# torchmd/torchmd-net

Measured on AMD Instinct MI355X. Metric: molecules/sec (64-atom molecules) TensorNet E+F, higher is better.
Workload: dtype f32; 1 GPU; BASELINE configs[1]: TensorNet F=128 L=2 K=32 rc=5.0, S-mol64 256 molecules x 64 atoms per GPU, energies + forces, random-init weights (seed 0); atoms_per_gpu=16384, pairs_per_gpu=193709, directed_edges_per_gpu=403802, parallelism=molecule-sharded x1, RCCL all-reduce of energies, rank_step=eager: tmdnet_build_graph (pair-count read-back) + tmdnet_energy_forces

## Files before the change

__graft_entry__.py:

```python
import os
import subprocess
import sys

ROOT = os.path.dirname(os.path.abspath(__file__))
PKG_DIR = os.path.join(ROOT, "torchmd-net_amd")
CSRC = os.path.join(PKG_DIR, "csrc")
LIB_DIR = os.path.join(PKG_DIR, "lib")
LIB = os.path.join(LIB_DIR, "libtmdnet_amd.so")
HIP_SOURCES = ["tn_api.hip", "tn_gemm.hip", "tn_gemm_skinny.hip", "tn_gemm_dual.hip", "tn_gemm_sb.hip", "tn_gemm_sb1.hip", "tn_tlin9.hip", "tn_small.hip", "tn_mid.hip", "tn_pairgrad.hip", "tn_kernels.hip", "tn_message_pair.hip", "tn_edge_table.hip", "tn_embed_rb.hip", "tn_train.hip", "tn_hvp.hip", "tn_et_hvp.hip", "tn_tn2_hvp.hip", "tn_hvp_api.hip", "tn_tn2.hip", "tn_tn2_api.hip", "tn_graph_wave.hip", "tn_neighbors_f64.hip", "tn_cell.hip", "tn_et.hip", "tn_et_g16.hip", "tn_et_api.hip", "tn_heads.hip", "tn_virial.hip"]

if PKG_DIR not in sys.path:
    sys.path.insert(0, PKG_DIR)
if ROOT not in sys.path:
    sys.path.insert(0, ROOT)


def _newer(target, sources):
    if not os.path.exists(target):
        return True
    t = os.path.getmtime(target)
    return any(os.path.getmtime(s) > t for s in sources)


def build_hip(force=False, verbose=True):
    from concurrent.futures import ThreadPoolExecutor

    os.makedirs(LIB_DIR, exist_ok=True)
    obj_dir = os.path.join(PKG_DIR, "build")
    os.makedirs(obj_dir, exist_ok=True)
    srcs = [os.path.join(CSRC, s) for s in HIP_SOURCES]
    headers = [os.path.join(CSRC, h) for h in os.listdir(CSRC) if h.endswith(".h")]
    headers.append(os.path.join(ROOT, "include", "tmdnet_amd.h"))
    hipcc = os.environ.get("HIPCC", "/opt/rocm/bin/hipcc")
    flags = ["--offload-arch=gfx950", "-O3", "-std=c++17", "-fPIC", "-Wno-unused-value", "-I" + os.path.join(ROOT, "include")]
    objs, todo = [], []
    for src in srcs:
        obj = os.path.join(obj_dir, os.path.basename(src)[:-4] + ".o")
        objs.append(obj)
        if force or _newer(obj, [src] + headers):
            todo.append((src, obj))

    def compile_one(job):
        src, obj = job
        cmd = [hipcc] + flags + ["-c", src, "-o", obj]
        if verbose:
            print("[build]", " ".join(cmd), flush=True)
        subprocess.check_call(cmd)

    if todo:
# ... 54 lines not shown
```

torchmd-net_amd/csrc/tn_api.hip:

```cpp
#include <hip/hip_runtime.h>

#include <algorithm>
#include <cmath>
#include <cstdio>
#include <cstdlib>
#include <cstring>
#include <map>
#include <unordered_map>
#include <string>
#include <vector>

#include "tn_heads.h"
#include "tn_model.h"
#include "tn_tlin9.h"
#include "tn_small.h"
#include "tn_interp.h"
#include "tn_virial.h"

using namespace tn;

static const char* kCatNames[CAT_COUNT] = {"graph", "gemm_edge", "gemm_node", "message", "pair_bwd", "embed_scatter", "elementwise", "edge_table"};

int fail(tmdnet_model* m, int code, const std::string& msg) {
  if (m) m->err = msg;
  return code;
}
// ... 872 lines not shown
      for (int l = 0; l <= L; ++l) {
        const std::string t = "cp" + std::to_string(l) + ".";
        add_sb(t + "W1", F, 3 * F);
        add_sb(t + "W1T", 3 * F, F);
        add_sb(t + "W2", F, F);
        add_sb(t + "W2T", F, F);
        add_sb(t + "W3", 2 * qd, F);
        add_sb(t + "W3T", F, 2 * qd);
      }
    }
    add_sb("Lin", F, 3 * F);
    add_sb("LinT", 3 * F, F);
    add_sb("O1", H, F);
    add_sb("O1T", F, H);
    std::vector<Img> fms;
    auto add_fm = [&](const std::string& key) {
      if (F % 32) return;
      fms.push_back({key, F, F, sb_elems});
      sb_elems += split_weight_fm_elems(F, F);
    };
    for (int k = 0; k < 3; ++k) {
      add_fm("Ue" + std::to_string(k));
      add_fm("UeT" + std::to_string(k));
    }
    for (int l = 0; l < L; ++l)
      for (int k = 0; k < 6; ++k) {
        add_fm("l" + std::to_string(l) + ".V" + std::to_string(k));
        add_fm("l" + std::to_string(l) + ".VT" + std::to_string(k));
      }
    if (m->dev_sb && m->dev_sb_cap < sb_elems) {
      HIP_TRY(m, hipFree(m->dev_sb));
      m->dev_sb = nullptr;
    }
    if (!m->dev_sb) {
      HIP_TRY(m, hipMalloc(reinterpret_cast<void**>(&m->dev_sb), sb_elems * sizeof(uint16_t)));
      m->dev_sb_cap = sb_elems;
    }
    for (const auto& im : imgs) launch_split_weight_tiles(m->dev + off.at(im.key), im.n, im.k, m->dev_sb + im.o, nullptr);
    for (const auto& im : fms) launch_split_weight_fm(m->dev + off.at(im.key), im.n, im.k, m->dev_sb + im.o, nullptr);
    m->image_jobs.clear();
    for (const auto& im : imgs) m->image_jobs.push_back({off.at(im.key), im.n, im.k, im.o, 0});
    for (const auto& im : fms) m->image_jobs.push_back({off.at(im.key), im.n, im.k, im.o, 1});
    m->packed_elems = pk.buf.size();
    m->sb_of.clear();
// ... 131 lines not shown
  HIP_TRY(m, hipGetLastError());
  return TMDNET_OK;
}

int tmdnet_set_option(tmdnet_model* m, const char* name, double value) {
  if (!m || !name) return TMDNET_ERR_INVALID;
  const std::string n(name);
  if (n == "edge_table_min_pairs") {
    m->tab_min_pairs = value < 0 ? 0 : (int64_t)value;
    return TMDNET_OK;
  }
  if (n == "embed_rb_min_atoms") {
    m->rb_min_atoms = value < 0 ? 0 : (int64_t)value;
    return TMDNET_OK;
  }
  if (n == "pair_rows_bf16") {
    if (!m->et) return fail(m, TMDNET_ERR_INVALID, "pair_rows_bf16 applies to the Equivariant Transformer handle only");
    m->pair_bf16 = value != 0.0 ? 1 : 0;
    return TMDNET_OK;
  }
  if (n == "recompute_pair_rows") {
    if (m->et || m->tn2) return fail(m, TMDNET_ERR_INVALID, "recompute_pair_rows applies to the TensorNet handle only");
    m->recompute_rows = value != 0.0;
    return TMDNET_OK;
  }
  return fail(m, TMDNET_ERR_INVALID, "unknown option: " + n);
}

int tmdnet_get_info(const tmdnet_model* m, const char* name, double* value) {
  if (!m || !name || !value) return TMDNET_ERR_INVALID;
  const std::string n(name);
  if (m->tabs_pending && n.rfind("edge_table_", 0) == 0 && n != "edge_table_min_pairs")
    if (const int rc = ensure_radial_tables(const_cast<tmdnet_model*>(m), nullptr)) return rc;
  if (n == "edge_table_T") *value = m->tabs.ok ? m->tabs.T : 0;
  else if (n == "edge_table_err_value") *value = m->tabs.err_value;
  else if (n == "edge_table_err_slope") *value = m->tabs.err_slope;
  else if (n == "edge_table_min_pairs") *value = (double)m->tab_min_pairs;
  else if (n == "pair_rows_bf16") *value = (double)m->pair_bf16;
  else if (n == "embed_rb_min_atoms") *value = (double)m->rb_min_atoms;
  else if (n == "recompute_pair_rows") *value = m->recompute_rows ? 1.0 : 0.0;
  else if (n == "embed_rb") *value = m->rb_fwd ? 1.0 : 0.0;
  else if (n == "species_last_build") *value = (double)m->last_nt;
  else if (n == "halo_active_first") *value = (double)m->halo_active[0];
  else if (n == "halo_active_rows") *value = (double)m->halo_active[1];
  else return TMDNET_ERR_INVALID;
  return TMDNET_OK;
}

int tmdnet_set_cell_grid(tmdnet_model* m, int32_t ncx, int32_t ncy, int32_t ncz) {
  if (!m) return TMDNET_ERR_INVALID;
  if (ncx < 0 || ncy < 0 || ncz < 0) ncx = ncy = ncz = -1;
  m->cell_n[0] = ncx;
  m->cell_n[1] = ncy;
  m->cell_n[2] = ncz;
// ... 307 lines not shown
    if (h[2] > 0 && h[2] < N && h[1] - h[0] + 1 == h[2] && images && tlin9_ok(h[2], F, true)) {
      a0 = h[0];
      Na = h[2];
    }
  }
  const bool rng = Na != N;
  const bool t9 = !tc && tlin9_ok(Na, F, rng) && tlin9_images(W.Ue) && tlin9_images(W.UeT) && (L == 0 || tlin9_images(W.layer[0].V));
  const bool t9r = !tc && L > 0 && tlin9_ok(Na, F, rng) && tlin9_images(W.UeT) && tlin9_images(W.layer[0].VT);
  m->halo_active[0] = a0;
  m->halo_active[1] = Na;
  const int64_t o1_ = a0, oF = (int64_t)a0 * F, o2F = 2 * oF, o3F = 3 * oF, o9F = 9 * oF, oH = (int64_t)a0 * H;
  const float* const q_a = q ? q + o1_ : nullptr;
  const int64_t* const batch_a = batch_k ? batch_k + o1_ : nullptr;
  const bool fused_small = !tc && !ntp && !recompute && !m->halo_fn && !m->head_kind && (small_fused_ok(N, F, H, L) || mid_fused_ok(N, F, H, L)) &&
                           (!want_forces || (message_adjoint_gd_ok(N, F) && !getenv("TMDNET_SEPARATE_PAIR_GD")));
  if (run_fwd) {
    if (use_tab) {
      const float* tabs[8];
      float* outs[8];
      float* douts[8];
      int nt_ = 0;
      if (!ntp) {
        tabs[nt_] = m->tabs.tab[0];
        outs[nt_] = b.Q;
        douts[nt_++] = want_forces ? b.dQ : nullptr;
      }
      for (int l = 0; l < L && !recompute; ++l) {
        tabs[nt_] = m->tabs.tab[1 + l];
        outs[nt_] = b.w[l];
        douts[nt_++] = want_forces ? b.dw[l] : nullptr;
// ... 66 lines not shown
        la.bO2 = W.bO2; la.atomref = W.atomref; la.Lin = W.Lin; la.O1 = W.O1; la.std_ = W.std;
        la.xhr = b.xhr; la.rstdr = b.rstdr; la.al = b.al; la.x = b.x; la.ea = b.ea;
        if (want_forces) { la.G = b.G; la.gMi = b.gMi; la.gPn = b.gPn; }
        KR(CAT_MESSAGE, wB + idxB + 6 * nodeB, (use_mid ? launch_mid_layer(la, last, s) : launch_small_layer(la, last, s)));
      }
      if (!want_forces) KR(CAT_ELEMENTWISE, Nd * 4, launch_mol_sum(g, b.ea, batch, N, B, W.mean, energy, s));
    } else {
    if (ntp) {
      KR(CAT_SCATTER, E_ * 12 + Pd * 48 + momB,
         (launch_pair_scalars(g, P, hp.cutoff_lower, hp.cutoff_upper, b.ps, s), launch_embed_moments(g, N, rbp, ntp, b.ps, b.mom, s)));
      KR(CAT_SCATTER, momB + Nd * 10 * Fd * 4, launch_embed_combine(g, N, F, K, ntp, z, W.Utab, W.Vtab, m->rb_fwd, b.mom, b.u0, b.s0n, s));
    } else {
      KR(CAT_SCATTER, Pd * 12 * Fd + E_ * 12 + Nd * 10 * Fd * 4,
         launch_embed_scatter(g, N, F, z, W.Utab, W.Vtab, b.Q, b.C, b.u0, b.s0n, s));
    }
    KR(CAT_ELEMENTWISE, Nd * Fd * 12,
       launch_layernorm_fwd(b.s0n + oF, W.ln0_w, W.ln0_b, Na, F, b.ln0 + oF, b.xh0 + oF, b.rstd0 + o1_, s));
    NODE();
    gemm(s, b.ln0 + oF, F, W.L1, F, W.bL1, b.h1 + o2F, 2 * F, Na, 2 * F, F, GEMM_ACT_SILU, b.a1 + o2F, 2 * F);
    gemm(s, b.h1 + o2F, 2 * F, W.L2, 2 * F, W.bL2, b.gates + o3F, 3 * F, Na, 3 * F, 2 * F, GEMM_ACT_SILU, b.a2 + o3F, 3 * F);
    if (t9) {
      Tl9Args ta{};
      ta.A = b.u0 + o9F; ta.C = b.X[0] + o9F; ta.o1 = b.UX + o9F; ta.e3 = b.gates + o3F; ta.N = Na; ta.F = F;
      tlin9(s, TL9_PRO_PLAIN, TL9_EPI_MULGATE, W.Ue, ta, 3.0 + 1.0 / 3.0, "gate");
    } else
      tensor_linear(s, b.u0, W.Ue, b.X[0], N, F, GEMM_MUL_AUX, b.UX, b.gates);
    for (int l = 0; l < L; ++l) {
      const LayerP& q_ = W.layer[l];
      if (es != s) HIP_TRY(m, hipStreamWaitEvent(s, m->ev_join[l], 0));
      float* const Xh_l = tc ? tc->Xh[l] : b.Xh;
      float* const Ch_l = tc ? tc->Ch[l] : b.Ch;
      float* const Xh_n = tc && l + 1 < L ? tc->Xh[l + 1] : b.Xh;
      if (t9) {
        Tl9Args ta{};
        ta.A = b.X[l] + o9F; ta.C = b.Pn[l] + o9F; ta.N = Na; ta.F = F;
// ... 5 lines not shown
        tb.A = Ch_l + o9F; tb.C = b.D[l] + o9F; tb.e0 = b.X[l] + o9F; tb.o1 = b.X[l + 1] + o9F; tb.o2 = b.feat + o3F;
        tb.want_feat = l + 1 == L; tb.kap = q_a;
        tb.N = Na; tb.F = F;
        tlin9(s, TL9_PRO_PLAIN, TL9_EPI_UPDATE, q_.V + 3, tb, 4.0 + (l + 1 == L ? 1.0 / 3.0 : 0.0), "update");
        continue;
      }
      if (l == 0) KR(CAT_ELEMENTWISE, 2 * nodeB, launch_norm_x(b.X[l], Xh_l, N, F, s));
      tensor_linear(s, Xh_l, q_.V, b.Pn[l], N, F);
      HALO_TRY(l, b.Pn[l], 9 * F);
      KR(CAT_MESSAGE, wB + idxB + 3 * nodeB, launch_message(g, N, F, b.w[l], b.Pn[l], q, batch_k, o3, b.Mi[l], Ch_l, s, recompute ? &rts[l] : nullptr));
      tensor_linear(s, Ch_l, q_.V + 3, b.D[l], N, F);
      KR(CAT_ELEMENTWISE, 4 * nodeB, launch_layer_update(Xh_l, b.D[l], q, batch_k, N, F, b.X[l + 1], l + 1 < L ? 1 : 2,
                                                         l + 1 < L ? Xh_n : b.feat, s));
    }
    if (L == 0) KR(CAT_ELEMENTWISE, nodeB + Nd * 3 * Fd * 4, launch_readout_feat(b.X[L] + o9F, Na, F, b.feat + o3F, s));
    KR(CAT_ELEMENTWISE, Nd * 3 * Fd * 12,
       launch_layernorm_fwd(b.feat + o3F, W.lnr_w, W.lnr_b, Na, 3 * F, b.lnr + o3F, b.xhr + o3F, b.rstdr + o1_, s));
    NODE();
    gemm(s, b.lnr + o3F, 3 * F, W.Lin, 3 * F, W.bLin, b.x + oF, F, Na, F, 3 * F, GEMM_ACT_SILU, b.al + oF, F);
    gemm(s, b.x + oF, F, W.O1, F, W.bO1, b.ao + oH, H, Na, H, F);
    if (m->head_kind) {
      KR(CAT_ELEMENTWISE, Nd * H * 4,
         launch_head_energy(b.ao, W.O2, W.bO2, N, H, W.std, nullptr, z, b.ea, s, want_forces ? b.g_ao : nullptr));
      heads.state = want_forces ? hbuf.state : nullptr;
      KR(CAT_ELEMENTWISE, Nd * 32, launch_heads_reduce(g, heads, hbuf, s));
    } else if ((int64_t)N <= 256 * (int64_t)B) {
      KR(CAT_ELEMENTWISE, Nd * H * 4, launch_head_mol_sum(g, b.ao, W.O2, W.bO2, N, B, H, W.std, W.atomref, z, batch, W.mean, energy, s,
                                                          want_forces ? b.g_ao : nullptr, m->atom_w, perm));
    } else {
      if (Na != N) launch_fill(b.ea, 0.f, N, s);
      KR(CAT_ELEMENTWISE, Nd * H * 4,
         launch_head_energy(b.ao + oH, W.O2, W.bO2, Na, H, W.std, W.atomref, z + o1_, b.ea + o1_, s, want_forces ? b.g_ao + oH : nullptr,
                            perm ? m->atom_w : (m->atom_w ? m->atom_w + o1_ : nullptr), perm ? perm + o1_ : nullptr));
      KR(CAT_ELEMENTWISE, Nd * 4, launch_mol_sum(g, b.ea, batch, N, B, W.mean, energy, s));
    }
    }
  }
  if (m->head_kind && want_forces && run_bwd)
    KR(CAT_ELEMENTWISE, Nd * (8 * H + 40), launch_heads_seed(heads, H, b.g_ao, hbuf.direct, s));

  if (want_forces && run_bwd && fused_small) {
    const int gd_nw = message_adjoint_gd_waves(g, N, F, recompute);
    const int64_t gd_stride = 2 * (int64_t)P1;
    for (int l = L - 1; l >= 0; --l) {
      const LayerP& q_ = W.layer[l];
      float* const gMi_in = ((L - 1 - l) & 1) ? b.gCh : b.gMi;
      float* const gMi_out = ((L - 1 - l) & 1) ? b.gMi : b.gCh;
      SmallRevArgs ra{};
      ra.g = g; ra.N = N; ra.F = F; ra.B = B; ra.o3 = o3; ra.first = l == 0; ra.kap = q;
// ... 22 lines not shown
    const RowMap rH = rows_plain(H), rF = rows_plain(F), r2F = rows_plain(2 * F), r3F = rows_plain(3 * F), rK = rows_plain(K);
    const RowMap rc_[3] = {rows_comp(F, 1), rows_comp(F, 3), rows_comp(F, 5)};
    const int c0_[3] = {0, 1, 4}, nc_[3] = {1, 3, 5};
    auto tensor_linear_grad = [&](const float* gOut, const float* In, const std::string& key) {
      for (int t = 0; t < 3; ++t)
        launch_tn_gemm(s, gOut + (int64_t)c0_[t] * F, rc_[t], In + (int64_t)c0_[t] * F, rc_[t], nullptr, nullptr, N * nc_[t], F, F,
                       tc->at(key + std::to_string(t)), false, tc->part);
    };
    if (tc) {
      launch_train_seed(b.ao, tc->gE, batch, N, H, W.std, b.g_ao, tc->head, s);
      launch_colsum(s, tc->head, rows_plain(H + 1), nullptr, rH, nullptr, nullptr, N, H, tc->at("O2"), false, tc->part);
      launch_colsum(s, tc->head + H, rows_plain(H + 1), nullptr, rH, nullptr, nullptr, N, 1, tc->at("bO2"), false, tc->part);
      launch_tn_gemm(s, b.g_ao, rH, b.x, rF, nullptr, nullptr, N, H, F, tc->at("O1"), false, tc->part);
      launch_colsum(s, b.g_ao, rH, nullptr, rH, nullptr, nullptr, N, H, tc->at("bO1"), false, tc->part);
    }
    gemm(s, b.g_ao + oH, H, W.O1T, H, nullptr, b.g_al + oF, F, Na, F, H, GEMM_MUL_DSILU_AUX, nullptr, 0, b.al + oF, F);
    gemm(s, b.g_al + oF, F, W.LinT, F, nullptr, b.g_ln + o3F, 3 * F, Na, 3 * F, F);
    if (tc) {
      launch_tn_gemm(s, b.g_al, rF, b.lnr, r3F, nullptr, nullptr, N, F, 3 * F, tc->at("Lin"), false, tc->part);
      launch_colsum(s, b.g_al, rF, nullptr, rF, nullptr, nullptr, N, F, tc->at("bLin"), false, tc->part);
      launch_colsum(s, b.g_ln, r3F, b.xhr, r3F, nullptr, nullptr, N, 3 * F, tc->at("lnr_w"), false, tc->part);
      launch_colsum(s, b.g_ln, r3F, nullptr, r3F, nullptr, nullptr, N, 3 * F, tc->at("lnr_b"), false, tc->part);
    }
    if (F % 64 == 0) {
      KR(CAT_ELEMENTWISE, 2 * nodeB + Nd * 3 * Fd * 8,
         launch_lnbwd_readout_bwd(b.g_ln + o3F, b.xhr + o3F, b.rstdr + o1_, W.lnr_w, Na, F, b.X[L] + o9F, b.G + o9F, s));
    } else {
      KR(CAT_ELEMENTWISE, Nd * 3 * Fd * 12,
         launch_layernorm_bwd(b.g_ln + o3F, b.xhr + o3F, b.rstdr + o1_, W.lnr_w, Na, 3 * F, b.g_feat + o3F, s));
      KR(CAT_ELEMENTWISE, 2 * nodeB + Nd * 3 * Fd * 4, launch_readout_bwd(b.X[L] + o9F, b.g_feat + o3F, Na, F, b.G + o9F, s));
    }
    const bool merged_gd = message_adjoint_gd_ok(N, F) && !getenv("TMDNET_SEPARATE_PAIR_GD") && !tc;
    const int gd_nw = message_adjoint_gd_waves(g, N, F, recompute);
    const int64_t gd_stride = 2 * (int64_t)P1;
    if (!merged_gd) launch_fill(b.gd, 0.f, P1, s);
    for (int l = L - 1; l >= 0; --l) {
      const LayerP& q_ = W.layer[l];
      if (t9r) {
        Tl9Args ta{};
// ... 45 lines not shown
        }
        continue;
      }
      if (tc) tensor_linear_grad(b.gPn, tc->Xh[l], "l" + std::to_string(l) + ".V"  + std::string("a"));
      tensor_linear(s, b.gPn, q_.VT, b.gXl, N, F);
      if (l > 0)
        KR(CAT_ELEMENTWISE, 6 * nodeB, launch_norm_bwd_update_bwd(b.X[l], b.gXl, N, F, b.G, b.D[l - 1], q, batch_k, b.gD, s));
      else
        KR(CAT_ELEMENTWISE, 5 * nodeB + Nd * 3 * Fd * 12,
           launch_norm_bwd_gate_bwd(b.X[0], b.gXl, N, F, b.G, b.UX, b.gates, b.a2, b.gUX, b.g_a2, s));
    }
    if (L == 0)
      KR(CAT_ELEMENTWISE, 3 * nodeB + Nd * 3 * Fd * 12,
         launch_embed_gate_bwd(b.G + o9F, b.UX + o9F, b.gates + o3F, b.a2 + o3F, Na, F, b.gUX + o9F, b.g_a2 + o3F, s));
    NODE();
    gemm(s, b.g_a2 + o3F, 3 * F, W.L2T, 3 * F, nullptr, b.g_a1 + o2F, 2 * F, Na, 2 * F, 3 * F, GEMM_MUL_DSILU_AUX, nullptr, 0, b.a1 + o2F, 2 * F);
    gemm(s, b.g_a1 + o2F, 2 * F, W.L1T, 2 * F, nullptr, b.g_ln0 + oF, F, Na, F, 2 * F);
    KR(CAT_ELEMENTWISE, Nd * Fd * 12, launch_layernorm_bwd(b.g_ln0 + oF, b.xh0 + oF, b.rstd0 + o1_, W.ln0_w, Na, F, b.g_s0n + oF, s));
    if (!tc && tlin9_ok(Na, F, rng) && tlin9_images(W.UeT)) {
      Tl9Args ta{};
      ta.A = b.gUX + o9F; ta.e0 = b.u0 + o9F; ta.e1 = b.g_s0n + oF; ta.o1 = b.gA + 10 * oF; ta.N = Na; ta.F = F;
      tlin9(s, TL9_PRO_PLAIN, TL9_EPI_EMBBWD, W.UeT, ta, 2.0 + 11.0 / 9.0, "embbwd");
    } else {
      tensor_linear(s, b.gUX, W.UeT, b.g_u0l, N, F);
      KR(CAT_ELEMENTWISE, 2 * nodeB + Nd * 11 * Fd * 4, launch_embed_bwd_atom(b.g_u0l, b.u0, b.g_s0n, N, F, b.gA, s));
    }
    HALO_TRY(200, b.gA, 10 * F);
    if (tc) {
      tensor_linear_grad(b.gUX, b.u0, "Ue");
      launch_tn_gemm(s, b.g_a2, r3F, b.h1, r2F, nullptr, nullptr, N, 3 * F, 2 * F, tc->at("L2"), false, tc->part);
      launch_colsum(s, b.g_a2, r3F, nullptr, r3F, nullptr, nullptr, N, 3 * F, tc->at("bL2"), false, tc->part);
      launch_tn_gemm(s, b.g_a1, r2F, b.ln0, rF, nullptr, nullptr, N, 2 * F, F, tc->at("L1"), false, tc->part);
      launch_colsum(s, b.g_a1, r2F, nullptr, r2F, nullptr, nullptr, N, 2 * F, tc->at("bL1"), false, tc->part);
// ... 331 lines not shown
```

torchmd-net_amd/csrc/tn_model.h:

```cpp
#pragma once
#include <hip/hip_runtime.h>

#include <cstdio>
#include <cstring>
#include <map>
#include <string>
#include <unordered_map>
#include <vector>

#include "../../include/tmdnet_amd.h"
#include "tn_gemm.h"
#include "tn_kernels.h"
#include "tn_train.h"

using namespace tn;


struct LayerP {
  const float *M1, *b1, *M2, *b2, *M3, *b3;
  const float *M2T, *M3T;
  const float* V[6];
  const float* VT[6];
  const uint16_t* M_sb[3];
};
// ... 155 lines not shown
  std::unordered_map<const float*, const uint16_t*> sb_of;
  std::unordered_map<const float*, const uint16_t*> fm_of;
  struct ImageJob { size_t src_off; int64_t n, k; size_t dst_off; int fm; };
  std::vector<ImageJob> image_jobs;
  size_t packed_elems = 0;
  int32_t* upd_tid = nullptr;
  int32_t* upd_ofs = nullptr;
  const float** upd_ptrs = nullptr;
  bool upd_ready = false;
  DevParams P;
  EdgeTables tabs;
  uint16_t* rb_img = nullptr;
  const uint16_t *rb_fwd = nullptr, *rb_rev = nullptr;
  int last_nt = 0;
  int64_t rb_min_atoms = 1024;
  int pair_bf16 = 0;
  bool tabs_pending = false;
  int64_t tab_min_pairs = 1;
  bool finalized = false;
  std::string err;
  FwdBuffers last{};
  int64_t lastN = 0, lastP = 0;
  bool has_last = false;
  const float* tn2_last_chg = nullptr;
};


int fail(tmdnet_model* m, int code, const std::string& msg);
#define HIP_TRY(m, expr)                                                                    \
  do {                                                                                      \
// ... 94 lines not shown
```

Baseline: 100,800 molecules/s.

## Fuse gate MLP and readout head chains into single split-bf16 MFMA kernels

Adds three fused kernels that chain layernorm, two GEMMs and SiLU activations through shared memory: the embedding gate forward, the gate backward, and the readout forward+backward head. Each keeps a 32-atom row tile in LDS as split-bf16 planes and runs 3-pass bf16 MFMA against pre-split weight images, replacing several separate GEMM and elementwise launches and their global intermediate round-trips. New fm weight images are built for Lin, O1, L1, L2 and their transposes. It is enabled only for F=128 (H=64 for the readout) with N at least 4096 atoms. The tile uses a lot of LDS per block, which may limit occupancy. The build script also gains an early return when the library is up to date.

```diff
diff --git a/__graft_entry__.py b/__graft_entry__.py
--- a/__graft_entry__.py
+++ b/__graft_entry__.py
@@ -7,7 +7,7 @@
 CSRC = os.path.join(PKG_DIR, "csrc")
 LIB_DIR = os.path.join(PKG_DIR, "lib")
 LIB = os.path.join(LIB_DIR, "libtmdnet_amd.so")
-HIP_SOURCES = ["tn_api.hip", "tn_gemm.hip", "tn_gemm_skinny.hip", "tn_gemm_dual.hip", "tn_gemm_sb.hip", "tn_gemm_sb1.hip", "tn_tlin9.hip", "tn_small.hip", "tn_mid.hip", "tn_pairgrad.hip", "tn_kernels.hip", "tn_message_pair.hip", "tn_edge_table.hip", "tn_embed_rb.hip", "tn_train.hip", "tn_hvp.hip", "tn_et_hvp.hip", "tn_tn2_hvp.hip", "tn_hvp_api.hip", "tn_tn2.hip", "tn_tn2_api.hip", "tn_graph_wave.hip", "tn_neighbors_f64.hip", "tn_cell.hip", "tn_et.hip", "tn_et_g16.hip", "tn_et_api.hip", "tn_heads.hip", "tn_virial.hip"]
+HIP_SOURCES = ["tn_api.hip", "tn_gemm.hip", "tn_gemm_skinny.hip", "tn_gemm_dual.hip", "tn_gemm_sb.hip", "tn_gemm_sb1.hip", "tn_tlin9.hip", "tn_chain.hip", "tn_small.hip", "tn_mid.hip", "tn_pairgrad.hip", "tn_kernels.hip", "tn_message_pair.hip", "tn_edge_table.hip", "tn_embed_rb.hip", "tn_train.hip", "tn_hvp.hip", "tn_et_hvp.hip", "tn_tn2_hvp.hip", "tn_hvp_api.hip", "tn_tn2.hip", "tn_tn2_api.hip", "tn_graph_wave.hip", "tn_neighbors_f64.hip", "tn_cell.hip", "tn_et.hip", "tn_et_g16.hip", "tn_et_api.hip", "tn_heads.hip", "tn_virial.hip"]
 
 if PKG_DIR not in sys.path:
     sys.path.insert(0, PKG_DIR)
@@ -33,6 +33,8 @@
     headers.append(os.path.join(ROOT, "include", "tmdnet_amd.h"))
     hipcc = os.environ.get("HIPCC", "/opt/rocm/bin/hipcc")
     flags = ["--offload-arch=gfx950", "-O3", "-std=c++17", "-fPIC", "-Wno-unused-value", "-I" + os.path.join(ROOT, "include")]
+    if not force and os.path.exists(LIB) and not _newer(LIB, srcs + headers):
+        return LIB
     objs, todo = [], []
     for src in srcs:
         obj = os.path.join(obj_dir, os.path.basename(src)[:-4] + ".o")
diff --git a/torchmd-net_amd/csrc/tn_api.hip b/torchmd-net_amd/csrc/tn_api.hip
--- a/torchmd-net_amd/csrc/tn_api.hip
+++ b/torchmd-net_amd/csrc/tn_api.hip
@@ -10,6 +10,7 @@
 #include <string>
 #include <vector>
 
+#include "tn_chain.h"
 #include "tn_heads.h"
 #include "tn_model.h"
 #include "tn_tlin9.h"
@@ -912,20 +913,32 @@
     add_sb("O1", H, F);
     add_sb("O1T", F, H);
     std::vector<Img> fms;
-    auto add_fm = [&](const std::string& key) {
-      if (F % 32) return;
-      fms.push_back({key, F, F, sb_elems});
-      sb_elems += split_weight_fm_elems(F, F);
+    auto add_fm = [&](const std::string& key, int64_t n, int64_t k) {
+      if ((n % 32) || (k % 16)) return;
+      fms.push_back({key, n, k, sb_elems});
+      sb_elems += split_weight_fm_elems(n, k);
     };
     for (int k = 0; k < 3; ++k) {
-      add_fm("Ue" + std::to_string(k));
-      add_fm("UeT" + std::to_string(k));
+      add_fm("Ue" + std::to_string(k), F, F);
+      add_fm("UeT" + std::to_string(k), F, F);
     }
     for (int l = 0; l < L; ++l)
       for (int k = 0; k < 6; ++k) {
-        add_fm("l" + std::to_string(l) + ".V" + std::to_string(k));
-        add_fm("l" + std::to_string(l) + ".VT" + std::to_string(k));
-      }
+        add_fm("l" + std::to_string(l) + ".V" + std::to_string(k), F, F);
+        add_fm("l" + std::to_string(l) + ".VT" + std::to_string(k), F, F);
+      }
+    if (!m->tn2 && chain_readout_shape_ok(F, H)) {
+      add_fm("Lin", F, 3 * F);
+      add_fm("LinT", 3 * F, F);
+      add_fm("O1", H, F);
+      add_fm("O1T", F, H);
+    }
+    if (!m->tn2 && chain_gate_shape_ok(F)) {
+      add_fm("L1", 2 * F, F);
+      add_fm("L2", 3 * F, 2 * F);
+      add_fm("L2T", 2 * F, 3 * F);
+      add_fm("L1T", F, 2 * F);
+    }
     if (m->dev_sb && m->dev_sb_cap < sb_elems) {
       HIP_TRY(m, hipFree(m->dev_sb));
       m->dev_sb = nullptr;
@@ -1087,6 +1100,14 @@
     m->rb_min_atoms = value < 0 ? 0 : (int64_t)value;
     return TMDNET_OK;
   }
+  if (n == "chain_min_atoms") {
+    m->chain_min_atoms = value < 0 ? 0 : (value > 9e18 ? INT64_MAX : (int64_t)value);
+    return TMDNET_OK;
+  }
+  if (n == "chain_mask") {
+    m->chain_mask = (int)value & 7;
+    return TMDNET_OK;
+  }
   if (n == "pair_rows_bf16") {
     if (!m->et) return fail(m, TMDNET_ERR_INVALID, "pair_rows_bf16 applies to the Equivariant Transformer handle only");
     m->pair_bf16 = value != 0.0 ? 1 : 0;
@@ -1111,6 +1132,9 @@
   else if (n == "edge_table_min_pairs") *value = (double)m->tab_min_pairs;
   else if (n == "pair_rows_bf16") *value = (double)m->pair_bf16;
   else if (n == "embed_rb_min_atoms") *value = (double)m->rb_min_atoms;
+  else if (n == "chain_min_atoms") *value = (double)m->chain_min_atoms;
+  else if (n == "chain_mask") *value = (double)m->chain_mask;
+  else if (n == "chain_last") *value = (double)m->chain_last;
   else if (n == "recompute_pair_rows") *value = m->recompute_rows ? 1.0 : 0.0;
   else if (n == "embed_rb") *value = m->rb_fwd ? 1.0 : 0.0;
   else if (n == "species_last_build") *value = (double)m->last_nt;
@@ -1448,6 +1472,17 @@
   const int64_t* const batch_a = batch_k ? batch_k + o1_ : nullptr;
   const bool fused_small = !tc && !ntp && !recompute && !m->halo_fn && !m->head_kind && (small_fused_ok(N, F, H, L) || mid_fused_ok(N, F, H, L)) &&
                            (!want_forces || (message_adjoint_gd_ok(N, F) && !getenv("TMDNET_SEPARATE_PAIR_GD")));
+  auto fm_image = [&](const float* w) -> const uint16_t* {
+    auto it = m->fm_of.find(w);
+    return it == m->fm_of.end() ? nullptr : it->second;
+  };
+  const bool chain_any = !tc && !m->head_kind && !m->halo_fn && Na == N && !fused_small && (int64_t)N >= m->chain_min_atoms;
+  const bool chain_ro = chain_any && (m->chain_mask & 1) && want_forces && run_fwd && run_bwd && chain_readout_shape_ok(F, H) &&
+                        fm_image(W.Lin) && fm_image(W.LinT) && fm_image(W.O1) && fm_image(W.O1T);
+  const bool chain_gate = chain_any && want_forces && run_fwd && run_bwd && chain_gate_shape_ok(F);
+  const bool chain_gf = chain_gate && (m->chain_mask & 2) && fm_image(W.L1) && fm_image(W.L2);
+  const bool chain_gb = chain_gate && (m->chain_mask & 4) && fm_image(W.L2T) && fm_image(W.L1T);
+  m->chain_last = (chain_ro ? 1 : 0) | (chain_gf ? 2 : 0) | (chain_gb ? 4 : 0);
   if (run_fwd) {
     if (use_tab) {
       const float* tabs[8];
@@ -1544,11 +1579,21 @@
       KR(CAT_SCATTER, Pd * 12 * Fd + E_ * 12 + Nd * 10 * Fd * 4,
          launch_embed_scatter(g, N, F, z, W.Utab, W.Vtab, b.Q, b.C, b.u0, b.s0n, s));
     }
+    NODE();
+    if (chain_gf) {
+      ChainGateFwdArgs ca{};
+      ca.s0n = b.s0n; ca.xh0 = b.xh0; ca.rstd0 = b.rstd0; ca.a1 = b.a1; ca.a2 = b.a2; ca.gates = b.gates;
+      ca.ln_w = W.ln0_w; ca.ln_b = W.ln0_b; ca.bL1 = W.bL1; ca.bL2 = W.bL2; ca.L1_fm = fm_image(W.L1); ca.L2_fm = fm_image(W.L2); ca.N = N;
+      char lab[64];
+      std::snprintf(lab, sizeof(lab), "chain gate_fwd %dx%d", N, F);
+      ProfScope ps_(s, CAT_GEMM_NODE, 2.0 * Nd * 8.0 * Fd * Fd, Nd * 10 * Fd * 4 + Nd * 4 + 4.0 * 8.0 * Fd * Fd, lab);
+      if (launch_chain_gate_fwd(ca, F, s)) return fail(m, TMDNET_ERR_HIP, "launch_chain_gate_fwd");
+    } else {
     KR(CAT_ELEMENTWISE, Nd * Fd * 12,
        launch_layernorm_fwd(b.s0n + oF, W.ln0_w, W.ln0_b, Na, F, b.ln0 + oF, b.xh0 + oF, b.rstd0 + o1_, s));
-    NODE();
     gemm(s, b.ln0 + oF, F, W.L1, F, W.bL1, b.h1 + o2F, 2 * F, Na, 2 * F, F, GEMM_ACT_SILU, b.a1 + o2F, 2 * F);
     gemm(s, b.h1 + o2F, 2 * F, W.L2, 2 * F, W.bL2, b.gates + o3F, 3 * F, Na, 3 * F, 2 * F, GEMM_ACT_SILU, b.a2 + o3F, 3 * F);
+    }
     if (t9) {
       Tl9Args ta{};
       ta.A = b.u0 + o9F; ta.C = b.X[0] + o9F; ta.o1 = b.UX + o9F; ta.e3 = b.gates + o3F; ta.N = Na; ta.F = F;
@@ -1584,6 +1629,21 @@
                                                          l + 1 < L ? Xh_n : b.feat, s));
     }
     if (L == 0) KR(CAT_ELEMENTWISE, nodeB + Nd * 3 * Fd * 4, launch_readout_feat(b.X[L] + o9F, Na, F, b.feat + o3F, s));
+    if (chain_ro) {
+      ChainReadoutArgs ca{};
+      ca.feat = b.feat; ca.X = b.X[L]; ca.G = b.G; ca.x = b.x; ca.ea = b.ea;
+      ca.lnr_w = W.lnr_w; ca.lnr_b = W.lnr_b; ca.bLin = W.bLin; ca.bO1 = W.bO1; ca.O2 = W.O2; ca.bO2 = W.bO2;
+      ca.Lin_fm = fm_image(W.Lin); ca.LinT_fm = fm_image(W.LinT); ca.O1_fm = fm_image(W.O1); ca.O1T_fm = fm_image(W.O1T);
+      ca.atomref = W.atomref; ca.z = z; ca.aw = m->atom_w; ca.perm = perm; ca.std_ = W.std; ca.N = N;
+      {
+        char lab[64];
+        std::snprintf(lab, sizeof(lab), "chain readout_fb %dx%dx%d", N, F, H);
+        ProfScope ps_(s, CAT_GEMM_NODE, 2.0 * Nd * (2.0 * 3 * Fd * Fd + 2.0 * Fd * H),
+                      2 * nodeB + Nd * 4 * Fd * 4 + Nd * 4 + 4.0 * (2.0 * 3 * Fd * Fd + 2.0 * Fd * H), lab);
+        if (launch_chain_readout_fb(ca, F, H, s)) return fail(m, TMDNET_ERR_HIP, "launch_chain_readout_fb");
+      }
+      KR(CAT_ELEMENTWISE, Nd * 4, launch_mol_sum(g, b.ea, batch, N, B, W.mean, energy, s));
+    } else {
     KR(CAT_ELEMENTWISE, Nd * 3 * Fd * 12,
        launch_layernorm_fwd(b.feat + o3F, W.lnr_w, W.lnr_b, Na, 3 * F, b.lnr + o3F, b.xhr + o3F, b.rstdr + o1_, s));
     NODE();
@@ -1603,6 +1663,7 @@
          launch_head_energy(b.ao + oH, W.O2, W.bO2, Na, H, W.std, W.atomref, z + o1_, b.ea + o1_, s, want_forces ? b.g_ao + oH : nullptr,
                             perm ? m->atom_w : (m->atom_w ? m->atom_w + o1_ : nullptr), perm ? perm + o1_ : nullptr));
       KR(CAT_ELEMENTWISE, Nd * 4, launch_mol_sum(g, b.ea, batch, N, B, W.mean, energy, s));
+    }
     }
     }
   }
@@ -1655,15 +1716,16 @@
       launch_tn_gemm(s, b.g_ao, rH, b.x, rF, nullptr, nullptr, N, H, F, tc->at("O1"), false, tc->part);
       launch_colsum(s, b.g_ao, rH, nullptr, rH, nullptr, nullptr, N, H, tc->at("bO1"), false, tc->part);
     }
-    gemm(s, b.g_ao + oH, H, W.O1T, H, nullptr, b.g_al + oF, F, Na, F, H, GEMM_MUL_DSILU_AUX, nullptr, 0, b.al + oF, F);
-    gemm(s, b.g_al + oF, F, W.LinT, F, nullptr, b.g_ln + o3F, 3 * F, Na, 3 * F, F);
+    if (!chain_ro) gemm(s, b.g_ao + oH, H, W.O1T, H, nullptr, b.g_al + oF, F, Na, F, H, GEMM_MUL_DSILU_AUX, nullptr, 0, b.al + oF, F);
+    if (!chain_ro) gemm(s, b.g_al + oF, F, W.LinT, F, nullptr, b.g_ln + o3F, 3 * F, Na, 3 * F, F);
     if (tc) {
       launch_tn_gemm(s, b.g_al, rF, b.lnr, r3F, nullptr, nullptr, N, F, 3 * F, tc->at("Lin"), false, tc->part);
       launch_colsum(s, b.g_al, rF, nullptr, rF, nullptr, nullptr, N, F, tc->at("bLin"), false, tc->part);
       launch_colsum(s, b.g_ln, r3F, b.xhr, r3F, nullptr, nullptr, N, 3 * F, tc->at("lnr_w"), false, tc->part);
       launch_colsum(s, b.g_ln, r3F, nullptr, r3F, nullptr, nullptr, N, 3 * F, tc->at("lnr_b"), false, tc->part);
     }
-    if (F % 64 == 0) {
+    if (chain_ro) {
+    } else if (F % 64 == 0) {
       KR(CAT_ELEMENTWISE, 2 * nodeB + Nd * 3 * Fd * 8,
          launch_lnbwd_readout_bwd(b.g_ln + o3F, b.xhr + o3F, b.rstdr + o1_, W.lnr_w, Na, F, b.X[L] + o9F, b.G + o9F, s));
     } else {
@@ -1739,9 +1801,19 @@
       KR(CAT_ELEMENTWISE, 3 * nodeB + Nd * 3 * Fd * 12,
          launch_embed_gate_bwd(b.G + o9F, b.UX + o9F, b.gates + o3F, b.a2 + o3F, Na, F, b.gUX + o9F, b.g_a2 + o3F, s));
     NODE();
+    if (chain_gb) {
+      ChainGateBwdArgs ca{};
+      ca.g_a2 = b.g_a2; ca.a1 = b.a1; ca.xh0 = b.xh0; ca.rstd0 = b.rstd0; ca.ln_w = W.ln0_w; ca.g_s0n = b.g_s0n;
+      ca.L2T_fm = fm_image(W.L2T); ca.L1T_fm = fm_image(W.L1T); ca.N = N;
+      char lab[64];
+      std::snprintf(lab, sizeof(lab), "chain gate_bwd %dx%d", N, F);
+      ProfScope ps_(s, CAT_GEMM_NODE, 2.0 * Nd * 8.0 * Fd * Fd, Nd * 7 * Fd * 4 + Nd * 4 + 4.0 * 8.0 * Fd * Fd, lab);
+      if (launch_chain_gate_bwd(ca, F, s)) return fail(m, TMDNET_ERR_HIP, "launch_chain_gate_bwd");
+    } else {
     gemm(s, b.g_a2 + o3F, 3 * F, W.L2T, 3 * F, nullptr, b.g_a1 + o2F, 2 * F, Na, 2 * F, 3 * F, GEMM_MUL_DSILU_AUX, nullptr, 0, b.a1 + o2F, 2 * F);
     gemm(s, b.g_a1 + o2F, 2 * F, W.L1T, 2 * F, nullptr, b.g_ln0 + oF, F, Na, F, 2 * F);
     KR(CAT_ELEMENTWISE, Nd * Fd * 12, launch_layernorm_bwd(b.g_ln0 + oF, b.xh0 + oF, b.rstd0 + o1_, W.ln0_w, Na, F, b.g_s0n + oF, s));
+    }
     if (!tc && tlin9_ok(Na, F, rng) && tlin9_images(W.UeT)) {
       Tl9Args ta{};
       ta.A = b.gUX + o9F; ta.e0 = b.u0 + o9F; ta.e1 = b.g_s0n + oF; ta.o1 = b.gA + 10 * oF; ta.N = Na; ta.F = F;
diff --git a/torchmd-net_amd/csrc/tn_chain.h b/torchmd-net_amd/csrc/tn_chain.h
--- /dev/null
+++ b/torchmd-net_amd/csrc/tn_chain.h
@@ -0,0 +1,44 @@
+#pragma once
+#include <hip/hip_runtime.h>
+#include <stdint.h>
+
+namespace tn {
+
+struct ChainReadoutArgs {
+  const float* feat;
+  const float* X;
+  float* G;
+  float* x;
+  float* ea;
+  const float *lnr_w, *lnr_b, *bLin, *bO1, *O2, *bO2;
+  const uint16_t *Lin_fm, *LinT_fm, *O1_fm, *O1T_fm;
+  const float* atomref;
+  const int64_t* z;
+  const float* aw;
+  const int* perm;
+  float std_;
+  int N;
+};
+
+struct ChainGateFwdArgs {
+  const float* s0n;
+  float *xh0, *rstd0;
+  float *a1, *a2, *gates;
+  const float *ln_w, *ln_b, *bL1, *bL2;
+  const uint16_t *L1_fm, *L2_fm;
+  int N;
+};
+struct ChainGateBwdArgs {
+  const float *g_a2, *a1, *xh0, *rstd0, *ln_w;
+  float* g_s0n;
+  const uint16_t *L2T_fm, *L1T_fm;
+  int N;
+};
+
+bool chain_readout_shape_ok(int F, int H);
+bool chain_gate_shape_ok(int F);
+int launch_chain_readout_fb(const ChainReadoutArgs& a, int F, int H, hipStream_t s);
+int launch_chain_gate_fwd(const ChainGateFwdArgs& a, int F, hipStream_t s);
+int launch_chain_gate_bwd(const ChainGateBwdArgs& a, int F, hipStream_t s);
+
+}
diff --git a/torchmd-net_amd/csrc/tn_chain.hip b/torchmd-net_amd/csrc/tn_chain.hip
--- /dev/null
+++ b/torchmd-net_amd/csrc/tn_chain.hip
@@ -0,0 +1,476 @@
+#include <cstdlib>
+
+#include "tn_chain.h"
+#include "tn_common.h"
+#include "tn_gemm_epi.h"
+#include "tn_gemm_sb.h"
+
+namespace tn {
+
+constexpr int CH_RA = 32;
+constexpr int CH_CS = 1024 + 32;
+constexpr int CH_D = 4;
+
+typedef float f2c __attribute__((ext_vector_type(2)));
+
+template <int NKC, int NACC>
+struct ChainMma {
+  static constexpr int STEPS = NKC * NACC;
+  bf16x8 wr[CH_D][3];
+  const uint16_t* wl;
+  int nbt, nb0, nbs;
+  __device__ __forceinline__ void fetch(int i) {
+    const int kc = i / NACC, j = i % NACC;
+    const uint16_t* p = wl + (int64_t)((kc * nbt + nb0 + j * nbs) * 3) * 512;
+#pragma unroll
+    for (int q = 0; q < 3; ++q) wr[i % CH_D][q] = *reinterpret_cast<const bf16x8*>(p + q * 512);
+  }
+  __device__ __forceinline__ void start(const uint16_t* img, int lane, int nbt_, int nb0_, int nbs_) {
+    wl = img + lane * 8;
+    nbt = nbt_;
+    nb0 = nb0_;
+    nbs = nbs_;
+#pragma unroll
+    for (int i = 0; i < CH_D; ++i)
+      if (i < STEPS) fetch(i);
+  }
+  __device__ __forceinline__ void run(const unsigned char* act, int pstride, floatx16 (&acc)[NACC]) {
+#pragma unroll
+    for (int j = 0; j < NACC; ++j)
+#pragma unroll
+      for (int e = 0; e < 16; ++e) acc[j][e] = 0.f;
+    bf16x8 af[2][3];
+#pragma unroll
+    for (int q = 0; q < 3; ++q) af[0][q] = *reinterpret_cast<const bf16x8*>(act + q * pstride);
+#pragma unroll
+    for (int kc = 0; kc < NKC; ++kc) {
+      if (kc + 1 < NKC) {
+#pragma unroll
+        for (int q = 0; q < 3; ++q) af[(kc + 1) & 1][q] = *reinterpret_cast<const bf16x8*>(act + q * pstride + (kc + 1) * CH_CS);
+      }
+#pragma unroll
+      for (int j = 0; j < NACC; ++j) {
+        const int i = kc * NACC + j;
+#define CH_MMA(pa_, pw_) acc[j] = __builtin_amdgcn_mfma_f32_32x32x16_bf16(wr[i % CH_D][pw_], af[kc & 1][pa_], acc[j], 0, 0, 0);
+        CH_MMA(0, 2) CH_MMA(2, 0) CH_MMA(1, 1) CH_MMA(0, 1) CH_MMA(1, 0) CH_MMA(0, 0)
+#undef CH_MMA
+        if (i + CH_D < STEPS) fetch(i + CH_D);
+        __builtin_amdgcn_sched_barrier(0);
+      }
+    }
+  }
+};
+
+__device__ __forceinline__ void chain_put4(unsigned char* base, int pstride, int r, int k, float v0, float v1, float v2, float v3) {
+  uint32_t h0, m0, l0, h1, m1, l1;
+  split2(v0, v1, h0, m0, l0);
+  split2(v2, v3, h1, m1, l1);
+  unsigned char* p = base + (k >> 4) * CH_CS + sb_piece(r, (k >> 3) & 1) + (k & 4) * 2;
+  *reinterpret_cast<uint2*>(p) = make_uint2(h0, h1);
+  *reinterpret_cast<uint2*>(p + pstride) = make_uint2(m0, m1);
+  *reinterpret_cast<uint2*>(p + 2 * pstride) = make_uint2(l0, l1);
+}
+
+template <int F, int H>
+__global__ __launch_bounds__(256, 2) void k_chain_readout_fb(ChainReadoutArgs a) {
+  static_assert(F == 128, "a lane holds channels 2 lane, 2 lane + 1 of each of the three invariants");
+  static_assert(H % 32 == 0 && H <= 128, "one wave per 32 head channels");
+  constexpr int R = 3 * F, NKL = R / 16, NKF = F / 16, NKH = H / 16;
+  constexpr int PL = NKL * CH_CS, PF = NKF * CH_CS, PH = NKH * CH_CS;
+  constexpr int O_X = 0, O_GAO = 3 * PF, O_GAL = O_GAO + 3 * PH, GLN_LD = R + 4, O_ES = 3 * PL;
+  static_assert(O_GAL + 3 * PF <= 3 * PL && CH_RA * GLN_LD * 4 <= 3 * PL, "stage buffers alias the first stage's planes");
+  __shared__ __attribute__((aligned(16))) unsigned char sm[3 * PL + CH_RA * 4];
+  float* const gln = reinterpret_cast<float*>(sm);
+  float* const es = reinterpret_cast<float*>(sm + O_ES);
+
+  const int tid = threadIdx.x, lane = tid & 63;
+  const int wave = __builtin_amdgcn_readfirstlane(tid >> 6);
+  const int N = a.N, m0 = blockIdx.x * CH_RA;
+  const int ra = lane & 31, hi = lane >> 5;
+  const int na = m0 + ra < N ? m0 + ra : N - 1;
+  const bool oka = m0 + ra < N;
+  const int frag = sb_piece(ra, hi);
+
+  f2c fx[8][3];
+  float rs[8];
+#pragma unroll
+  for (int i = 0; i < 8; ++i) {
+    const int n = m0 + wave * 8 + i;
+    const float* p = a.feat + (int64_t)(n < N ? n : N - 1) * R + 2 * lane;
+#pragma unroll
+    for (int t = 0; t < 3; ++t) fx[i][t] = *reinterpret_cast<const f2c*>(p + t * F);
+  }
+  f2c lw[3], lb[3];
+#pragma unroll
+  for (int t = 0; t < 3; ++t) {
+    lw[t] = *reinterpret_cast<const f2c*>(a.lnr_w + t * F + 2 * lane);
+    lb[t] = *reinterpret_cast<const f2c*>(a.lnr_b + t * F + 2 * lane);
+  }
+  ChainMma<NKL, 1> mm1;
+  mm1.start(a.Lin_fm, lane, F / 32, wave, 0);
+#pragma unroll
+  for (int i = 0; i < 8; ++i) {
+    float s = 0.f;
+#pragma unroll
+    for (int t = 0; t < 3; ++t) s += fx[i][t][0] + fx[i][t][1];
+    const float mean = wave_sum(s) / R;
+    float var = 0.f;
+#pragma unroll
+    for (int t = 0; t < 3; ++t) {
+      const float d0 = fx[i][t][0] - mean, d1 = fx[i][t][1] - mean;
+      var += d0 * d0 + d1 * d1;
+    }
+    var = wave_sum(var) / R;
+    rs[i] = 1.0f / sqrtf(var + 1e-5f);
+    const int r = wave * 8 + i;
+#pragma unroll
+    for (int t = 0; t < 3; ++t) {
+      fx[i][t] = (fx[i][t] - mean) * rs[i];
+      const f2c y = fx[i][t] * lw[t] + lb[t];
+      uint32_t h, m, l;
+      split2(y[0], y[1], h, m, l);
+      unsigned char* p = sm + (t * NKF + (lane >> 3)) * CH_CS + sb_piece(r, (lane >> 2) & 1) + (lane & 3) * 4;
+      *reinterpret_cast<uint32_t*>(p) = h;
+      *reinterpret_cast<uint32_t*>(p + PL) = m;
+      *reinterpret_cast<uint32_t*>(p + 2 * PL) = l;
+    }
+  }
+  __syncthreads();
+
+  float al[16];
+  {
+    floatx16 acc[1];
+    mm1.run(sm + frag, PL, acc);
+    __syncthreads();
+#pragma unroll
+    for (int g = 0; g < 4; ++g) {
+      const int k = 32 * wave + 8 * g + 4 * hi;
+      const float4 b4 = *reinterpret_cast<const float4*>(a.bLin + k);
+      const float bb[4] = {b4.x, b4.y, b4.z, b4.w};
+      float xv[4];
+#pragma unroll
+      for (int e = 0; e < 4; ++e) {
+        al[4 * g + e] = acc[0][4 * g + e] + bb[e];
+        xv[e] = fast_silu(al[4 * g + e]);
+      }
+      if (oka) *reinterpret_cast<float4*>(a.x + (int64_t)na * F + k) = make_float4(xv[0], xv[1], xv[2], xv[3]);
+      chain_put4(sm + O_X, PF, ra, k, xv[0], xv[1], xv[2], xv[3]);
+    }
+  }
+  __syncthreads();
+
+  const float wgt = a.aw ? a.aw[a.perm ? a.perm[na] : na] : 1.0f;
+  float esum = 0.f;
+  if (wave < H / 32) {
+    ChainMma<NKF, 1> mm2;
+    mm2.start(a.O1_fm, lane, H / 32, wave, 0);
+    floatx16 acc[1];
+    mm2.run(sm + O_X + frag, PF, acc);
+#pragma unroll
+    for (int g = 0; g < 4; ++g) {
+      const int k = 32 * wave + 8 * g + 4 * hi;
+      const float4 b4 = *reinterpret_cast<const float4*>(a.bO1 + k), o4 = *reinterpret_cast<const float4*>(a.O2 + k);
+      const float bb[4] = {b4.x, b4.y, b4.z, b4.w}, oo[4] = {o4.x, o4.y, o4.z, o4.w};
+      float gv[4];
+#pragma unroll
+      for (int e = 0; e < 4; ++e) {
+        const float ao = acc[0][4 * g + e] + bb[e];
+        esum += silu(ao) * oo[e];
+        gv[e] = wgt * a.std_ * oo[e] * silu_grad(ao);
+      }
+      chain_put4(sm + O_GAO, PH, ra, k, gv[0], gv[1], gv[2], gv[3]);
+    }
+    esum += __shfl_xor(esum, 32, 64);
+    if (wave > 0 && lane < 32) es[(wave - 1) * CH_RA + ra] = esum;
+  }
+  ChainMma<NKH, 1> mm3;
+  mm3.start(a.O1T_fm, lane, F / 32, wave, 0);
+  __syncthreads();
+  if (wave == 0 && lane < 32 && oka) {
+    float s = esum;
+#pragma unroll
+    for (int w = 1; w < H / 32; ++w) s += es[(w - 1) * CH_RA + ra];
+    float e = (s + a.bO2[0]) * a.std_;
+    if (a.atomref) e += a.atomref[a.z[na]];
+    a.ea[na] = wgt * e;
+  }
+
+  {
+    floatx16 acc[1];
+    mm3.run(sm + O_GAO + frag, PH, acc);
+#pragma unroll
+    for (int g = 0; g < 4; ++g) {
+      float gv[4];
+#pragma unroll
+      for (int e = 0; e < 4; ++e) gv[e] = acc[0][4 * g + e] * fast_silu_grad(al[4 * g + e]);
+      chain_put4(sm + O_GAL, PF, ra, 32 * wave + 8 * g + 4 * hi, gv[0], gv[1], gv[2], gv[3]);
+    }
+  }
+  f2c xr[3][9];
+  auto load_x = [&](int i) __attribute__((always_inline)) {
+    const int n = m0 + wave * 8 + i;
+    const float* p = a.X + (int64_t)(n < N ? n : N - 1) * 9 * F + 2 * lane;
+#pragma unroll
+    for (int c = 0; c < 9; ++c) xr[i % 3][c] = *reinterpret_cast<const f2c*>(p + c * F);
+  };
+  ChainMma<NKF, 3> mm4;
+  mm4.start(a.LinT_fm, lane, R / 32, wave, 4);
+  __syncthreads();
+
+  {
+    floatx16 acc[3];
+    mm4.run(sm + O_GAL + frag, PF, acc);
+    load_x(0);
+    load_x(1);
+    __syncthreads();
+#pragma unroll
+    for (int j = 0; j < 3; ++j)
+#pragma unroll
+      for (int g = 0; g < 4; ++g)
+        *reinterpret_cast<float4*>(gln + ra * GLN_LD + 32 * (wave + 4 * j) + 8 * g + 4 * hi) =
+            make_float4(acc[j][4 * g], acc[j][4 * g + 1], acc[j][4 * g + 2], acc[j][4 * g + 3]);
+  }
+  load_x(2);
+  __syncthreads();
+
+#pragma unroll
+  for (int i = 0; i < 8; ++i) {
+    const int r = wave * 8 + i, n = m0 + r;
+    f2c gw[3];
+    float s1 = 0.f, s2 = 0.f;
+#pragma unroll
+    for (int t = 0; t < 3; ++t) {
+      gw[t] = *reinterpret_cast<const f2c*>(gln + r * GLN_LD + t * F + 2 * lane) * lw[t];
+      s1 += gw[t][0] + gw[t][1];
+      s2 += gw[t][0] * fx[i][t][0] + gw[t][1] * fx[i][t][1];
+    }
+    s1 = wave_sum(s1) / R;
+    s2 = wave_sum(s2) / R;
+    f2c gf[3];
+#pragma unroll
+    for (int t = 0; t < 3; ++t) gf[t] = (gw[t] - s1 - fx[i][t] * s2) * rs[i];
+    f2c o[9];
+#pragma unroll
+    for (int j = 0; j < 2; ++j) {
+      float u[9], dq[9];
+#pragma unroll
+      for (int c = 0; c < 9; ++c) u[c] = xr[i % 3][c][j];
+      dquad(u, dq);
+#pragma unroll
+      for (int c = 0; c < 9; ++c) o[c][j] = dq[c] * gf[type_of(c)][j];
+    }
+    if (i + 3 < 8) load_x(i + 3);
+    if (n < N) {
+      float* p = a.G + (int64_t)n * 9 * F + 2 * lane;
+#pragma unroll
+      for (int c = 0; c < 9; ++c) *reinterpret_cast<f2c*>(p + c * F) = o[c];
+    }
+  }
+}
+
+template <int F>
+__global__ __launch_bounds__(256, 2) void k_chain_gate_fwd(ChainGateFwdArgs a) {
+  static_assert(F == 128, "a lane holds channels 2 lane, 2 lane + 1 of the row");
+  constexpr int NK1 = F / 16, NK2 = 2 * F / 16;
+  constexpr int P1 = NK1 * CH_CS, P2 = NK2 * CH_CS, O_H = 3 * P1;
+  __shared__ __attribute__((aligned(16))) unsigned char sm[3 * P1 + 3 * P2];
+
+  const int tid = threadIdx.x, lane = tid & 63;
+  const int wave = __builtin_amdgcn_readfirstlane(tid >> 6);
+  const int N = a.N, m0 = blockIdx.x * CH_RA;
+  const int ra = lane & 31, hi = lane >> 5;
+  const int na = m0 + ra < N ? m0 + ra : N - 1;
+  const bool oka = m0 + ra < N;
+  const int frag = sb_piece(ra, hi);
+
+  f2c v[8];
+#pragma unroll
+  for (int i = 0; i < 8; ++i) {
+    const int n = m0 + wave * 8 + i;
+    v[i] = *reinterpret_cast<const f2c*>(a.s0n + (int64_t)(n < N ? n : N - 1) * F + 2 * lane);
+  }
+  const f2c lw = *reinterpret_cast<const f2c*>(a.ln_w + 2 * lane), lb = *reinterpret_cast<const f2c*>(a.ln_b + 2 * lane);
+  ChainMma<NK1, 2> mm1;
+  mm1.start(a.L1_fm, lane, 2 * F / 32, wave, 4);
+#pragma unroll
+  for (int i = 0; i < 8; ++i) {
+    const int r = wave * 8 + i, n = m0 + r;
+    const float mean = wave_sum(v[i][0] + v[i][1]) / F;
+    const float d0 = v[i][0] - mean, d1 = v[i][1] - mean;
+    const float var = wave_sum(d0 * d0 + d1 * d1) / F;
+    const float rs = 1.0f / sqrtf(var + 1e-5f);
+    const f2c xh = (v[i] - mean) * rs;
+    if (n < N) {
+      *reinterpret_cast<f2c*>(a.xh0 + (int64_t)n * F + 2 * lane) = xh;
+      if (lane == 0) a.rstd0[n] = rs;
+    }
+    const f2c y = xh * lw + lb;
+    uint32_t h, m, l;
+    split2(y[0], y[1], h, m, l);
+    unsigned char* p = sm + (lane >> 3) * CH_CS + sb_piece(r, (lane >> 2) & 1) + (lane & 3) * 4;
+    *reinterpret_cast<uint32_t*>(p) = h;
+    *reinterpret_cast<uint32_t*>(p + P1) = m;
+    *reinterpret_cast<uint32_t*>(p + 2 * P1) = l;
+  }
+  __syncthreads();
+
+  ChainMma<NK2, 3> mm2;
+  {
+    floatx16 acc[2];
+    mm1.run(sm + frag, P1, acc);
+    mm2.start(a.L2_fm, lane, 3 * F / 32, wave, 4);
+#pragma unroll
+    for (int j = 0; j < 2; ++j)
+#pragma unroll
+      for (int g = 0; g < 4; ++g) {
+        const int k = 32 * (wave + 4 * j) + 8 * g + 4 * hi;
+        const float4 b4 = *reinterpret_cast<const float4*>(a.bL1 + k);
+        const float p0 = acc[j][4 * g] + b4.x, p1 = acc[j][4 * g + 1] + b4.y, p2 = acc[j][4 * g + 2] + b4.z, p3 = acc[j][4 * g + 3] + b4.w;
+        if (oka) *reinterpret_cast<float4*>(a.a1 + (int64_t)na * 2 * F + k) = make_float4(p0, p1, p2, p3);
+        chain_put4(sm + O_H, P2, ra, k, fast_silu(p0), fast_silu(p1), fast_silu(p2), fast_silu(p3));
+      }
+  }
+  __syncthreads();
+
+  {
+    floatx16 acc[3];
+    mm2.run(sm + O_H + frag, P2, acc);
+    if (oka) {
+#pragma unroll
+      for (int j = 0; j < 3; ++j)
+#pragma unroll
+        for (int g = 0; g < 4; ++g) {
+          const int k = 32 * (wave + 4 * j) + 8 * g + 4 * hi;
+          const float4 b4 = *reinterpret_cast<const float4*>(a.bL2 + k);
+          const float p0 = acc[j][4 * g] + b4.x, p1 = acc[j][4 * g + 1] + b4.y, p2 = acc[j][4 * g + 2] + b4.z, p3 = acc[j][4 * g + 3] + b4.w;
+          *reinterpret_cast<float4*>(a.a2 + (int64_t)na * 3 * F + k) = make_float4(p0, p1, p2, p3);
+          *reinterpret_cast<float4*>(a.gates + (int64_t)na * 3 * F + k) = make_float4(fast_silu(p0), fast_silu(p1), fast_silu(p2), fast_silu(p3));
+        }
+    }
+  }
+}
+
+template <int F>
+__global__ __launch_bounds__(256, 2) void k_chain_gate_bwd(ChainGateBwdArgs a) {
+  static_assert(F == 128, "a lane holds channels 2 lane, 2 lane + 1 of the row");
+  constexpr int NK3 = 3 * F / 16, NK2 = 2 * F / 16;
+  constexpr int P3 = NK3 * CH_CS, P2 = NK2 * CH_CS;
+  constexpr int GL_LD = F + 4, O_GL = 3 * P2;
+  static_assert(O_GL + CH_RA * GL_LD * 4 <= 3 * P3, "stage buffers alias the first stage's planes");
+  __shared__ __attribute__((aligned(16))) unsigned char sm[3 * P3];
+  float* const gl = reinterpret_cast<float*>(sm + O_GL);
+
+  const int tid = threadIdx.x, lane = tid & 63;
+  const int wave = __builtin_amdgcn_readfirstlane(tid >> 6);
+  const int N = a.N, m0 = blockIdx.x * CH_RA;
+  const int ra = lane & 31, hi = lane >> 5;
+  const int na = m0 + ra < N ? m0 + ra : N - 1;
+  const int frag = sb_piece(ra, hi);
+
+  ChainMma<NK3, 2> mm1;
+  mm1.start(a.L2T_fm, lane, 2 * F / 32, wave, 4);
+  {
+    f2c v[8][3];
+#pragma unroll
+    for (int i = 0; i < 8; ++i) {
+      const int n = m0 + wave * 8 + i;
+      const float* p = a.g_a2 + (int64_t)(n < N ? n : N - 1) * 3 * F + 2 * lane;
+#pragma unroll
+      for (int t = 0; t < 3; ++t) v[i][t] = *reinterpret_cast<const f2c*>(p + t * F);
+    }
+#pragma unroll
+    for (int i = 0; i < 8; ++i)
+#pragma unroll
+      for (int t = 0; t < 3; ++t) {
+        uint32_t h, m, l;
+        split2(v[i][t][0], v[i][t][1], h, m, l);
+        unsigned char* p = sm + (t * (F / 16) + (lane >> 3)) * CH_CS + sb_piece(wave * 8 + i, (lane >> 2) & 1) + (lane & 3) * 4;
+        *reinterpret_cast<uint32_t*>(p) = h;
+        *reinterpret_cast<uint32_t*>(p + P3) = m;
+        *reinterpret_cast<uint32_t*>(p + 2 * P3) = l;
+      }
+  }
+  float4 a1v[2][4];
+#pragma unroll
+  for (int j = 0; j < 2; ++j)
+#pragma unroll
+    for (int g = 0; g < 4; ++g) a1v[j][g] = *reinterpret_cast<const float4*>(a.a1 + (int64_t)na * 2 * F + 32 * (wave + 4 * j) + 8 * g + 4 * hi);
+  __syncthreads();
+
+  ChainMma<NK2, 1> mm2;
+  {
+    floatx16 acc[2];
+    mm1.run(sm + frag, P3, acc);
+    mm2.start(a.L1T_fm, lane, F / 32, wave, 0);
+    __syncthreads();
+#pragma unroll
+    for (int j = 0; j < 2; ++j)
+#pragma unroll
+      for (int g = 0; g < 4; ++g) {
+        const float4 p = a1v[j][g];
+        chain_put4(sm, P2, ra, 32 * (wave + 4 * j) + 8 * g + 4 * hi, acc[j][4 * g] * fast_silu_grad(p.x), acc[j][4 * g + 1] * fast_silu_grad(p.y),
+                   acc[j][4 * g + 2] * fast_silu_grad(p.z), acc[j][4 * g + 3] * fast_silu_grad(p.w));
+      }
+  }
+  f2c xh[8];
+  float rs[8];
+#pragma unroll
+  for (int i = 0; i < 8; ++i) {
+    const int n = m0 + wave * 8 + i, nc = n < N ? n : N - 1;
+    xh[i] = *reinterpret_cast<const f2c*>(a.xh0 + (int64_t)nc * F + 2 * lane);
+    rs[i] = a.rstd0[nc];
+  }
+  const f2c lw = *reinterpret_cast<const f2c*>(a.ln_w + 2 * lane);
+  __syncthreads();
+
+  {
+    floatx16 acc[1];
+    mm2.run(sm + frag, P2, acc);
+#pragma unroll
+    for (int g = 0; g < 4; ++g)
+      *reinterpret_cast<float4*>(gl + ra * GL_LD + 32 * wave + 8 * g + 4 * hi) =
+          make_float4(acc[0][4 * g], acc[0][4 * g + 1], acc[0][4 * g + 2], acc[0][4 * g + 3]);
+  }
+  __syncthreads();
+
+#pragma unroll
+  for (int i = 0; i < 8; ++i) {
+    const int r = wave * 8 + i, n = m0 + r;
+    const f2c gw = *reinterpret_cast<const f2c*>(gl + r * GL_LD + 2 * lane) * lw;
+    const float s1 = wave_sum(gw[0] + gw[1]) / F;
+    const float s2 = wave_sum(gw[0] * xh[i][0] + gw[1] * xh[i][1]) / F;
+    if (n < N) *reinterpret_cast<f2c*>(a.g_s0n + (int64_t)n * F + 2 * lane) = (gw - s1 - xh[i] * s2) * rs[i];
+  }
+}
+
+static bool chain_off() {
+  static const bool off = getenv("TMDNET_NO_SPLIT_BF16") != nullptr;
+  return off;
+}
+bool chain_gate_shape_ok(int F) { return !chain_off() && F == 128; }
+
+int launch_chain_gate_fwd(const ChainGateFwdArgs& a, int F, hipStream_t s) {
+  if (!chain_gate_shape_ok(F)) return (int)hipErrorInvalidValue;
+  if (a.N <= 0) return 0;
+  hipLaunchKernelGGL((k_chain_gate_fwd<128>), dim3((a.N + CH_RA - 1) / CH_RA), dim3(256), 0, s, a);
+  return (int)hipGetLastError();
+}
+int launch_chain_gate_bwd(const ChainGateBwdArgs& a, int F, hipStream_t s) {
+  if (!chain_gate_shape_ok(F)) return (int)hipErrorInvalidValue;
+  if (a.N <= 0) return 0;
+  hipLaunchKernelGGL((k_chain_gate_bwd<128>), dim3((a.N + CH_RA - 1) / CH_RA), dim3(256), 0, s, a);
+  return (int)hipGetLastError();
+}
+
+bool chain_readout_shape_ok(int F, int H) {
+  return !chain_off() && F == 128 && H == 64;
+}
+
+int launch_chain_readout_fb(const ChainReadoutArgs& a, int F, int H, hipStream_t s) {
+  if (!chain_readout_shape_ok(F, H)) return (int)hipErrorInvalidValue;
+  if (a.N <= 0) return 0;
+  hipLaunchKernelGGL((k_chain_readout_fb<128, 64>), dim3((a.N + CH_RA - 1) / CH_RA), dim3(256), 0, s, a);
+  return (int)hipGetLastError();
+}
+
+}
diff --git a/torchmd-net_amd/csrc/tn_model.h b/torchmd-net_amd/csrc/tn_model.h
--- a/torchmd-net_amd/csrc/tn_model.h
+++ b/torchmd-net_amd/csrc/tn_model.h
@@ -193,6 +193,9 @@
   const uint16_t *rb_fwd = nullptr, *rb_rev = nullptr;
   int last_nt = 0;
   int64_t rb_min_atoms = 1024;
+  int64_t chain_min_atoms = 4096;
+  int chain_mask = 7;
+  int chain_last = 0;
   int pair_bf16 = 0;
   bool tabs_pending = false;
   int64_t tab_min_pairs = 1;
```

Result: faster. 105,700 molecules/s, median of 6 (+4.9%).
